# owensgroup/sparsify.me

Hardware: AMD Instinct MI355X
Metric: effective GF/s (2:4 spmma vs dense gemm) on ResNet-50 layer shapes (higher is better)
Workload: dtype f16

## Files before the change

sparsify.me_amd/csrc/spmma_f16_fused.hip:

```cpp
#include "select24.h"
#include "spmma_args.h"

namespace sm {

constexpr int MAXG = 8;
struct FusedArgs {
  const half_t* A[MAXG];
  const half_t* B[MAXG];
  half_t* C[MAXG];
  size_t sA, sB, sC;
  int Mrows, N, K, lda;
  int batch, tiles_m, tiles_n;
  int ngroup;
  float alpha, beta;
  const half_t* const* dAp;
  const half_t* const* dBp;
  half_t* const* dCp;
};

struct FusedArgsEpi : FusedArgs {
  EpiArgs e;
};
template <bool EPI> struct FusedArgsSel { typedef FusedArgs type; };
template <> struct FusedArgsSel<true> { typedef FusedArgsEpi type; };
// ... 568 lines not shown
  const int m0 = (int)tile_m * BM, n0 = (int)tile_n * BN;
  const int nkt = (p.K + 63) / 64;
  const char* A = reinterpret_cast<const char*>(p.dAp ? p.dAp[grp] : p.A[grp]);
  const half_t* B = p.dBp ? p.dBp[grp] : p.B[grp];
  half_t* C = p.dCp ? p.dCp[grp] : p.C[grp];
  const unsigned rowbytes = (unsigned)p.K * 2u;
  const int rows = p.Mrows - m0 < BM ? p.Mrows - m0 : BM;
  EpiBias<FM, FN> eb;
  if constexpr (EPI) eb = epi_bias_prefetch<FM, FN>(p.e, true, wave * TM, 0, m0, n0, p.Mrows, p.N, lane);

  {
    const size_t s0 = (size_t)m0 * rowbytes;
    const unsigned len = (unsigned)rows * rowbytes;
    const unsigned np = (len + 1023u) / 1024u;
    const size_t last16 = a_bytes - 16;
    for (unsigned pc = wave; pc < np; pc += NW) {
      size_t off = s0 + (size_t)pc * 1024u + 16u * lane;
      off = off < last16 ? off : last16;
      __builtin_amdgcn_global_load_lds((gptr_t*)(A + off), (lptr_t*)(smem + pc * 1024u), 16, 0, 2);
    }
  }
  char* const Bimg = smem + span_lds;
  {
    constexpr int B_N = BN / 8;
    const int npb = nkt * B_N;
    for (int t = (int)wave; t < npb; t += NW) {
      const int kt = t / B_N, j = t - kt * B_N;
      const unsigned panel = (unsigned)j >> 3, kr = 8u * ((unsigned)j & 7u) + (lane >> 3);
      const unsigned cs = (lane & 7u) ^ b_swz(kr);
      int gc = n0 + (int)(64u * panel + 8u * cs);
      gc = gc <= p.N - 8 ? gc : p.N - 8;
      const int krow = kt * 64 + (int)kr;
      const char* src = krow < p.K ? reinterpret_cast<const char*>(B + (size_t)krow * p.N + gc)
                                   : reinterpret_cast<const char*>(sm_fused_zero_page) + 16u * (lane & 7u);
      __builtin_amdgcn_global_load_lds((gptr_t*)src, (lptr_t*)(Bimg + kt * SB + panel * 8192u + ((unsigned)j & 7u) * 1024u), 16, 0, 0);
    }
  }
  wait_dma_and_barrier<0>();

  f4 acc[FM][FN];
#pragma unroll
  for (int i = 0; i < FM; ++i)
#pragma unroll
    for (int j = 0; j < FN; ++j) acc[i][j] = f4{0.f, 0.f, 0.f, 0.f};
  const unsigned g = lane >> 4, r = lane & 15u;
  unsigned rowoff[FM];
#pragma unroll
  for (int i = 0; i < FM; ++i) {
    int row = (int)(wave * TM + i * 16 + r);
    row = row < rows ? row : rows - 1;
    rowoff[i] = (unsigned)row * rowbytes;
  }
  for (int kt = 0; kt < nkt; ++kt) {
    if constexpr (DENSE) {
      h8 a0[FM], a1[FM];
#pragma unroll
      for (int i = 0; i < FM; ++i) {
        uint32_t d[2][4];
#pragma unroll
        for (int h = 0; h < 2; ++h) {
          const int k0 = kt * 64 + 32 * h + 8 * (int)g;
          int nv = p.K - k0;
          nv = nv < 0 ? 0 : (nv > 8 ? 8 : nv);
          const char* src = smem + rowoff[i] + 2u * (unsigned)k0;
#pragma unroll
          for (int e = 0; e < 4; ++e) {
            const uint32_t lo16 = *reinterpret_cast<const unsigned short*>(src + 4 * e);
            const uint32_t hi16 = *reinterpret_cast<const unsigned short*>(src + 4 * e + 2);
            uint32_t v = lo16 | (hi16 << 16);
            v = 2 * e + 1 < nv ? v : (2 * e < nv ? (v & 0xffffu) : 0u);
            d[h][e] = v;
          }
        }
        a0[i] = __builtin_bit_cast(h8, u4{d[0][0], d[0][1], d[0][2], d[0][3]});
        a1[i] = __builtin_bit_cast(h8, u4{d[1][0], d[1][1], d[1][2], d[1][3]});
      }
      mfma_b_sweep<FM, FN, BF>(a0, a1, Bimg + kt * SB, 0, lane, acc);
      continue;
    }
    h8 af[FM];
    int idx[FM];
    const int k0 = kt * 64 + 16 * (int)g;
    int nv = p.K - k0;
    nv = nv < 0 ? 0 : (nv > 16 ? 16 : nv);
#pragma unroll
    for (int i = 0; i < FM; ++i) {
      const char* src = smem + rowoff[i] + 2u * (unsigned)k0;
      uint32_t d[8];
#pragma unroll
      for (int e = 0; e < 8; ++e) {
        const uint32_t lo16 = *reinterpret_cast<const unsigned short*>(src + 4 * e);
        const uint32_t hi16 = *reinterpret_cast<const unsigned short*>(src + 4 * e + 2);
        uint32_t v = lo16 | (hi16 << 16);
        v = 2 * e + 1 < nv ? v : (2 * e < nv ? (v & 0xffffu) : 0u);
        d[e] = v;
      }
      dense16_to_operand(u4{d[0], d[1], d[2], d[3]}, u4{d[4], d[5], d[6], d[7]}, af[i], idx[i]);
    }
    smfmac_b_sweep<FM, FN, BF>(af, idx, Bimg + kt * SB, 0, lane, acc);
  }
  __syncthreads();
  if constexpr (EPI) store_c_tile_epi<BM, BN, FM, FN, 64 * NW, BF>(smem, C, p.e.R, p.e, eb, acc, true, wave * TM, 0, m0, n0, p.Mrows, p.N, p.alpha, p.beta, tid);
  else store_c_tile<BM, BN, FM, FN, 64 * NW, BF>(smem, C, acc, true, wave * TM, 0, m0, n0, p.Mrows, p.N, p.alpha, p.beta, tid);
}

template <int BN, bool BF = false, bool DENSE = false, bool EPI = false>
static int launch_fused_span(const typename FusedArgsSel<EPI>::type& a0, hipStream_t st) {
  typename FusedArgsSel<EPI>::type a = a0;
  a.tiles_m = (a.Mrows + 127) / 128;
  a.tiles_n = (a.N + BN - 1) / BN;
  const size_t nwg = (size_t)a.tiles_m * a.tiles_n * a.ngroup;
  if (nwg == 0) return SM_STATUS_SUCCESS;
  const size_t kc = ((size_t)a.K + 63) / 64 * 64;
  const size_t span_lds = ((size_t)128 * a.K * 2 + 128 + 1023) / 1024 * 1024;
  const size_t lds_main = span_lds + kc * BN * 2;
  constexpr size_t lds_epi = (size_t)128 * (BN * 2 + 16);
  const size_t lds = lds_main > lds_epi ? lds_main : lds_epi;
  if (lds > 160 * 1024 || nwg > 0x7fffffffu) {
    set_error("sm_spmma_fused_{f16,bf16}: k too long for the span form (use the staged path)");
    return SM_STATUS_NOT_SUPPORTED;
  }
  static LdsOptIn lds_optin;
  if (const int rc = ensure_dyn_lds(lds_optin, reinterpret_cast<const void*>(&spmma_f16_fused_span_kernel<BN, BF, DENSE, EPI>), 160 * 1024, "spmma_f16_fused_span_kernel")) return rc;
  spmma_f16_fused_span_kernel<BN, BF, DENSE, EPI><<<dim3((unsigned)nwg), dim3(256), lds, st>>>(a, (unsigned)span_lds, (size_t)a.Mrows * a.K * 2);
  return check_launch("spmma_f16_fused_span_kernel");
}

template <int BN, int NBW>
struct BTileDma {
  static constexpr int B_WI = (BN / 8) / NBW;
  const char* src[B_WI];
  unsigned dst[B_WI];
  size_t step;
  __device__ __forceinline__ void setup(const half_t* B, int N, int n0, unsigned bw, unsigned lane, unsigned ring_off) {
#pragma unroll
    for (int i = 0; i < B_WI; ++i) {
      const unsigned j = bw + (unsigned)NBW * i, panel = j >> 3, grp = j & 7u, kr = 8u * grp + (lane >> 3);
      const unsigned cs = (lane & 7u) ^ b_swz(kr);
      int gc = n0 + (int)(64u * panel + 8u * cs);
      gc = gc <= N - 8 ? gc : N - 8;
      src[i] = reinterpret_cast<const char*>(B) + ((size_t)kr * N + (size_t)gc) * 2;
      dst[i] = ring_off + panel * 8192u + grp * 1024u;
    }
    step = (size_t)64 * N * 2;
  }
  __device__ __forceinline__ void issue(char* smem, int kt, unsigned buf_off) const {
#pragma unroll
    for (int i = 0; i < B_WI; ++i)
      __builtin_amdgcn_global_load_lds((gptr_t*)(src[i] + (size_t)kt * step), (lptr_t*)(smem + buf_off + dst[i]), 16, 0, 0);
  }
};


template <int BN, int WM, int WN, int NLB, int PF, int NSB, bool BF = false, bool ANT = true, bool EPI = false>
__global__ __launch_bounds__(64 * (WM * WN + 4 + NLB)) void spmma_f16_fused_wide_kernel(const typename FusedArgsSel<EPI>::type p) {
  constexpr int BM = 128, NLA = 4, NC = WM * WN, NW = NC + NLA + NLB;
  static_assert(PF >= 1 && PF <= 3 && NSB >= 2 && NSB <= 4, "pipeline depths");
  constexpr int TM = BM / WM, TN = BN / WN, FM = TM / 16, FN = TN / 16;
  constexpr int SA = BM * 64, SM_ = BM * 8, ASTG = SA + SM_, SB = 64 * BN * 2;
  constexpr int BRING = 2 * ASTG;
  constexpr int NBW = NLB > 0 ? NLB : WM * WN;
  constexpr int B_N = BN / 8, B_WI = B_N / NBW;
  static_assert(B_N % NBW == 0 && B_WI >= 1 && (NSB - 2) * B_WI <= 63, "B tile vs issuing waves");
  extern __shared__ __attribute__((aligned(16))) char smem[];

  const unsigned tid = threadIdx.x, lane = tid & 63u;
  const unsigned wave = __builtin_amdgcn_readfirstlane(tid >> 6);
  const unsigned tiles = (unsigned)p.tiles_m * (unsigned)p.tiles_n;
  const unsigned lid = xcd_remap(blockIdx.x, gridDim.x);
  const unsigned gb = lid / tiles, trem = lid - gb * tiles;
  const unsigned grp = gb / (unsigned)p.batch, b = gb - grp * (unsigned)p.batch;
  const unsigned tile_m = trem / (unsigned)p.tiles_n, tile_n = trem - tile_m * (unsigned)p.tiles_n;
  const int m0 = (int)tile_m * BM, n0 = (int)tile_n * BN;
  const int nkt = p.K / 64;
  half_t* C = p.C[grp] + (size_t)b * p.sC;

  f4 acc[FM][FN];
#pragma unroll
  for (int i = 0; i < FM; ++i)
#pragma unroll
    for (int j = 0; j < FN; ++j) acc[i][j] = f4{0.f, 0.f, 0.f, 0.f};
  const unsigned wm = wave / WN, wn = wave % WN;
  EpiBias<FM, FN> eb;
  if constexpr (EPI) eb = epi_bias_prefetch<FM, FN>(p.e, wave < (unsigned)NC, wm * TM, wn * TN, m0, n0, p.Mrows, p.N, lane);

  if (NLB > 0 && wave >= (unsigned)(NC + NLA)) {
    BTileDma<BN, NBW> bd;
    bd.setup(p.B[grp] + (size_t)b * p.sB, p.N, n0, wave - (NC + NLA), lane, BRING);
    auto issue = [&](int kt, int buf) {
      bd.issue(smem, kt, (unsigned)(buf * SB));
    };
#pragma unroll
    for (int s = 0; s < NSB - 1; ++s)
      if (s < nkt) issue(s, s);
    int nb = NSB - 1;
    for (int kt = 0; kt < nkt; ++kt) {
      if (kt + NSB - 2 < nkt) wait_dma_and_barrier<(NSB - 2) * B_WI>();
      else wait_dma_and_barrier<0>();
      if (kt + NSB - 1 < nkt) {
        issue(kt + NSB - 1, nb);
        nb = nb + 1 == NSB ? 0 : nb + 1;
      }
    }
  } else if (wave >= (unsigned)NC) {
    const unsigned lw = wave - NC;
    const half_t* A = p.A[grp] + (size_t)b * p.sA;
    const int mlast = p.Mrows - 1;
    const unsigned c8 = lane & 7u;
    const half_t* a_src[4];
    unsigned a_val_off[4], a_meta_off[4];
#pragma unroll
    for (int i = 0; i < 4; ++i) {
      const unsigned row = 8u * (4u * lw + i) + (lane >> 3);
      int gr = m0 + (int)row;
      gr = gr < mlast ? gr : mlast;
      a_src[i] = A + (size_t)gr * p.lda + 8u * c8;
      a_val_off[i] = row * 64u + 16u * ((c8 >> 1) ^ a64_swz(row)) + 8u * (c8 & 1u);
      a_meta_off[i] = SA + row * 8u + c8;
    }
    u4 ra[PF][4];
    auto load_a = [&](int kt, u4 (&dst)[4]) {
#pragma unroll
      for (int i = 0; i < 4; ++i) {
        if constexpr (ANT) dst[i] = __builtin_nontemporal_load(reinterpret_cast<const u4*>(a_src[i] + (size_t)kt * 64));
        else dst[i] = *reinterpret_cast<const u4*>(a_src[i] + (size_t)kt * 64);
      }
      __builtin_amdgcn_sched_barrier(0);
    };
    auto write_stage = [&](int kt, const u4 (&src)[4]) {
      char* sb = smem + (kt & 1) * ASTG;
#pragma unroll
      for (int i = 0; i < 4; ++i) {
        uint32_t k0, k1, n0, n1;
        strip_select_f16(src[i][0], src[i][1], k0, n0);
        strip_select_f16(src[i][2], src[i][3], k1, n1);
        *reinterpret_cast<u2*>(sb + a_val_off[i]) = u2{k0, k1};
        *reinterpret_cast<unsigned char*>(sb + a_meta_off[i]) = (unsigned char)(n0 | (n1 << 4));
      }
    };
    auto step = [&](int kt, u4 (&rr)[4], bool write, bool load) {
      asm volatile("s_waitcnt lgkmcnt(0)\n\ts_barrier" ::: "memory");
      __builtin_amdgcn_sched_barrier(0);
      if (write) {
        write_stage(kt + 1, rr);
      }
      if (load) load_a(kt + 1 + PF, rr);
      __builtin_amdgcn_sched_barrier(0);
    };
    int kt0 = 0;
    if (nkt > 2 * PF) {
#pragma unroll
      for (int s = 0; s < PF; ++s) load_a(s, ra[s]);
      write_stage(0, ra[0]);
      load_a(PF, ra[0]);
      for (; kt0 + 2 * PF < nkt; kt0 += PF) {
#pragma unroll
        for (int u = 0; u < PF; ++u) step(kt0 + u, ra[(u + 1) % PF], true, true);
      }
    } else {
#pragma unroll
      for (int s = 0; s < PF; ++s)
        if (s < nkt) load_a(s, ra[s]);
      write_stage(0, ra[0]);
      if (PF < nkt) load_a(PF, ra[0]);
    }
    for (; kt0 < nkt; kt0 += PF) {
#pragma unroll
      for (int u = 0; u < PF; ++u) {
        const int kt = kt0 + u;
        if (kt < nkt) step(kt, ra[(u + 1) % PF], kt + 1 < nkt, kt + 1 + PF < nkt);
      }
    }
  } else {
    int cb = 0;
    BTileDma<BN, NBW> bd;
    int nb = NSB - 1;
    if (NLB == 0) {
      bd.setup(p.B[grp] + (size_t)b * p.sB, p.N, n0, wave, lane, BRING);
#pragma unroll
      for (int s = 0; s < NSB - 1; ++s)
        if (s < nkt) bd.issue(smem, s, (unsigned)(s * SB));
    }
    for (int kt = 0; kt < nkt; ++kt) {
      if (NLB == 0) {
        if (kt + NSB - 2 < nkt) wait_dma_and_barrier<(NSB - 2) * B_WI>();
        else wait_dma_and_barrier<0>();
        if (kt + NSB - 1 < nkt) {
          bd.issue(smem, kt + NSB - 1, (unsigned)(nb * SB));
          nb = nb + 1 == NSB ? 0 : nb + 1;
        }
      } else {
        wait_dma_and_barrier<0>();
      }
      const char* As = smem + (kt & 1) * ASTG;
      const char* Ms = As + SA;
      const char* Bs = smem + BRING + cb * SB;
      smfmac_stage<FM, FN, BF>(As, Ms, Bs, wm * TM, wn * TN, lane, acc);
      cb = cb + 1 == NSB ? 0 : cb + 1;
    }
  }
  __syncthreads();

  if constexpr (EPI) store_c_tile_epi<BM, BN, FM, FN, 64 * NW, BF>(smem, C, p.e.R + (size_t)b * p.e.sR, p.e, eb, acc, wave < (unsigned)NC, wm * TM, wn * TN, m0, n0, p.Mrows, p.N, p.alpha, p.beta, tid);
  else store_c_tile<BM, BN, FM, FN, 64 * NW, BF>(smem, C, acc, wave < (unsigned)NC, wm * TM, wn * TN, m0, n0, p.Mrows, p.N, p.alpha, p.beta, tid);
}

template <int BN, int WM, int WN, int NLB, int PF, int NSB, bool BF = false, bool ANT = true, bool EPI = false>
static int launch_fused_wide(const typename FusedArgsSel<EPI>::type& a0, hipStream_t st) {
  typename FusedArgsSel<EPI>::type a = a0;
  a.tiles_m = (a.Mrows + 127) / 128;
  a.tiles_n = (a.N + BN - 1) / BN;
  const size_t nwg = (size_t)a.tiles_m * a.tiles_n * a.batch * a.ngroup;
  if (nwg == 0) return SM_STATUS_SUCCESS;
  if (nwg > 0x7fffffffu) {
    set_error("sm_spmma_fused_f16: grid too large");
    return SM_STATUS_NOT_SUPPORTED;
  }
  constexpr size_t lds_main = 2 * (size_t)128 * 72 + (size_t)NSB * 64 * BN * 2;
  constexpr size_t lds_epi = (size_t)128 * (BN * 2 + 16);
  constexpr size_t lds = lds_main > lds_epi ? lds_main : lds_epi;
  static LdsOptIn lds_optin;
  if (lds > 64 * 1024) {
    if (const int rc = ensure_dyn_lds(lds_optin, reinterpret_cast<const void*>(&spmma_f16_fused_wide_kernel<BN, WM, WN, NLB, PF, NSB, BF, ANT, EPI>), lds, "spmma_f16_fused_wide_kernel")) return rc;
  }
  spmma_f16_fused_wide_kernel<BN, WM, WN, NLB, PF, NSB, BF, ANT, EPI><<<dim3((unsigned)nwg), dim3(64 * (WM * WN + 4 + NLB)), lds, st>>>(a);
  return check_launch("spmma_f16_fused_wide_kernel");
}

template <int BN, int WM, int WN, int NLB, int PF, int NSB, bool BF = false>
__global__ __launch_bounds__(64 * (WM * WN + 4 + NLB)) void spmma_f16_fused_widep_kernel(const FusedArgs p, const unsigned total) {
  constexpr int BM = 128, NLA = 4, NC = WM * WN;
  static_assert(NLB > 0 && PF >= 1 && PF <= 3 && NSB >= 2 && NSB <= 4, "pipeline depths");
  constexpr int TM = BM / WM, TN = BN / WN, FM = TM / 16, FN = TN / 16;
  static_assert(TN == 128 && TM == 32, "epilogue patch geometry");
  constexpr int SA = BM * 64, SM_ = BM * 8, ASTG = SA + SM_, SB = 64 * BN * 2;
  constexpr int BRING = 2 * ASTG;
  constexpr int B_N = BN / 8, B_WI = B_N / NLB;
  static_assert(B_N % NLB == 0 && (NSB - 2) * B_WI <= 63, "B tile vs loader waves");
  constexpr int WPITCH = 64 * 2 + 8, WPATCH = TM * WPITCH;
  constexpr int CPATCH = BRING + NSB * SB;
  extern __shared__ __attribute__((aligned(16))) char smem[];

  const unsigned tid = threadIdx.x, lane = tid & 63u;
  const unsigned wave = __builtin_amdgcn_readfirstlane(tid >> 6);
  const unsigned tiles = (unsigned)p.tiles_m * (unsigned)p.tiles_n;
  const int nkt = p.K / 64;
  const unsigned my_tiles = (total - blockIdx.x + gridDim.x - 1u) / gridDim.x;
  const int S = (int)my_tiles * nkt;

  struct Tile {
    unsigned grp, b;
    int m0, n0;
  };
  auto tile_of = [&](unsigned j) {
    Tile t;
    const unsigned lid = xcd_remap(blockIdx.x + j * gridDim.x, total);
    const unsigned gb = lid / tiles, trem = lid - gb * tiles;
    t.grp = gb / (unsigned)p.batch;
    t.b = gb - t.grp * (unsigned)p.batch;
    const unsigned tile_m = trem / (unsigned)p.tiles_n, tile_n = trem - tile_m * (unsigned)p.tiles_n;
    t.m0 = (int)tile_m * BM;
    t.n0 = (int)tile_n * BN;
    return t;
  };

  if (wave >= (unsigned)(NC + NLA)) {
    BTileDma<BN, NLB> bd;
    unsigned ij = 0;
    int ikt = 0, nb = 0;
    {
      const Tile t = tile_of(0);
      bd.setup(p.B[t.grp] + (size_t)t.b * p.sB, p.N, t.n0, wave - (NC + NLA), lane, BRING);
    }
    auto issue = [&]() {
      bd.issue(smem, ikt, (unsigned)(nb * SB));
      nb = nb + 1 == NSB ? 0 : nb + 1;
      if (++ikt == nkt) {
        ikt = 0;
        if (++ij < my_tiles) {
          const Tile t = tile_of(ij);
          bd.setup(p.B[t.grp] + (size_t)t.b * p.sB, p.N, t.n0, wave - (NC + NLA), lane, BRING);
        }
      }
    };
#pragma unroll
    for (int s = 0; s < NSB - 1; ++s)
      if (s < S) issue();
    for (int g = 0; g < S; ++g) {
      if (g + NSB - 2 < S) wait_dma_and_barrier<(NSB - 2) * B_WI>();
      else wait_dma_and_barrier<0>();
      if (g + NSB - 1 < S) issue();
    }
  } else if (wave >= (unsigned)NC) {
    const unsigned lw = wave - NC;
    const unsigned c8 = lane & 7u;
    const half_t* a_src[4];
    unsigned a_val_off[4], a_meta_off[4];
#pragma unroll
    for (int i = 0; i < 4; ++i) {
      const unsigned row = 8u * (4u * lw + i) + (lane >> 3);
      a_val_off[i] = row * 64u + 16u * ((c8 >> 1) ^ a64_swz(row)) + 8u * (c8 & 1u);
      a_meta_off[i] = SA + row * 8u + c8;
    }
    const int mlast = p.Mrows - 1;
    auto point_at = [&](unsigned j) {
      const Tile t = tile_of(j);
      const half_t* A = p.A[t.grp] + (size_t)t.b * p.sA;
#pragma unroll
      for (int i = 0; i < 4; ++i) {
        const unsigned row = 8u * (4u * lw + i) + (lane >> 3);
        int gr = t.m0 + (int)row;
        gr = gr < mlast ? gr : mlast;
        a_src[i] = A + (size_t)gr * p.lda + 8u * c8;
      }
    };
    point_at(0);
    unsigned lj = 0;
    int lkt = 0;
    u4 ra[PF][4];
    auto load_a = [&](u4 (&dst)[4]) {
#pragma unroll
      for (int i = 0; i < 4; ++i) dst[i] = __builtin_nontemporal_load(reinterpret_cast<const u4*>(a_src[i] + (size_t)lkt * 64));
      __builtin_amdgcn_sched_barrier(0);
      if (++lkt == nkt) {
        lkt = 0;
        if (++lj < my_tiles) point_at(lj);
      }
    };
    auto write_stage = [&](int g, const u4 (&src)[4]) {
      char* sb = smem + (g & 1) * ASTG;
#pragma unroll
      for (int i = 0; i < 4; ++i) {
        uint32_t k0, k1, n0, n1;
        strip_select_f16(src[i][0], src[i][1], k0, n0);
        strip_select_f16(src[i][2], src[i][3], k1, n1);
        *reinterpret_cast<u2*>(sb + a_val_off[i]) = u2{k0, k1};
        *reinterpret_cast<unsigned char*>(sb + a_meta_off[i]) = (unsigned char)(n0 | (n1 << 4));
      }
    };
    auto step = [&](int g, u4 (&rr)[4], bool write, bool load) {
      asm volatile("s_waitcnt lgkmcnt(0)\n\ts_barrier" ::: "memory");
      __builtin_amdgcn_sched_barrier(0);
      if (write) write_stage(g + 1, rr);
      if (load) load_a(rr);
      __builtin_amdgcn_sched_barrier(0);
    };
    int g0 = 0;
    if (S > 2 * PF) {
#pragma unroll
      for (int s = 0; s < PF; ++s) load_a(ra[s]);
      write_stage(0, ra[0]);
      load_a(ra[0]);
      for (; g0 + 2 * PF < S; g0 += PF) {
#pragma unroll
        for (int u = 0; u < PF; ++u) step(g0 + u, ra[(u + 1) % PF], true, true);
      }
    } else {
#pragma unroll
      for (int s = 0; s < PF; ++s)
        if (s < S) load_a(ra[s]);
      write_stage(0, ra[0]);
      if (PF < S) load_a(ra[0]);
    }
    for (; g0 < S; g0 += PF) {
#pragma unroll
      for (int u = 0; u < PF; ++u) {
        const int g = g0 + u;
        if (g < S) step(g, ra[(u + 1) % PF], g + 1 < S, g + 1 + PF < S);
      }
    }
  } else {
    const unsigned g4 = lane >> 4, r = lane & 15u;
    const unsigned wm = wave / WN, wn = wave % WN;
    char* const patch = smem + CPATCH + wave * WPATCH;
    f4 acc[FM][FN];
#pragma unroll
    for (int i = 0; i < FM; ++i)
#pragma unroll
// ... 263 lines not shown
using namespace sm;

static bool span_form_takes(size_t m, size_t n, size_t k, size_t lda, size_t batch, size_t strideA, size_t strideB, size_t strideC, bool all_aligned, bool c_aligned) {
  return (k % 64 != 0 || lda % 8 != 0) && lda == k && n % 8 == 0 && n <= 128 && all_aligned && c_aligned && (batch == 1 || (strideB == 0 && strideA == m * lda && strideC == m * n)) &&
         (m * batch * k * 2) % 16 == 0 && m * batch <= 0x7fffffffull && k <= 0x7fffffffull &&
         ((size_t)128 * k * 2 + 1152) + ((k + 63) / 64 * 64) * (n <= 64 ? 64 : 128) * 2 <= 160 * 1024;
}
static bool stage_forms_take(size_t n, size_t k, size_t lda, size_t strideA, size_t strideB, bool all_aligned) {
  return !(k % 64 != 0 || lda % 8 != 0 || strideA % 8 != 0 || n % 8 != 0 || strideB % 8 != 0 || !all_aligned);
}
static bool dims_fit_int(size_t m, size_t n, size_t k, size_t lda, size_t batch) {
  return !(m * batch > 0x7fffffffull || n > 0x7fffffffull || k > 0x7fffffffull || lda > 0x7fffffffull);
}

struct FusedCall {
  size_t m, n, k, lda, batch, count, sA, sB, sC;
  float beta;
  bool a_aligned, b_aligned, c_aligned;
  bool ws, ws_aligned;
  size_t ws_bytes;
  bool epi, r_aligned;
  size_t sR;
};
struct FusedPick {
  int form;
  bool stacked;
  const char* why;
};

static FusedPick fused_form(const FusedCall& c, size_t cus) {
  const size_t m = c.m, n = c.n, k = c.k, lda = c.lda, batch = c.batch;
  if (c.count == 0 || m == 0 || n == 0 || batch == 0) return {SM_FUSED_FORM_EMPTY, false, nullptr};
  const bool all_aligned = c.a_aligned && c.b_aligned;
  const bool contiguous = c.sB == 0 && c.sA == m * lda && c.sC == m * n;
  if (n < 8 && k <= 64 && lda == k && (batch == 1 || contiguous)) {
    if (c.epi) return {SM_FUSED_FORM_NOT_TAKEN, false, "sm_spmma_fused_{f16,bf16}_ex: the thin form (n < 8) takes no epilogue"};
    if (thin_form_takes(c.count, m * batch, n, k) && c.a_aligned) return {SM_FUSED_FORM_THIN, true, nullptr};
  }
  const bool r_follows = !c.epi || c.beta == 0.0f || (c.r_aligned && (batch == 1 || c.sR == m * n));
  if (span_form_takes(m, n, k, lda, batch, c.sA, c.sB, c.sC, all_aligned, c.c_aligned && r_follows)) return {SM_FUSED_FORM_SPAN, true, nullptr};
  if (!stage_forms_take(n, k, lda, c.sA, c.sB, all_aligned))
    return {SM_FUSED_FORM_NOT_TAKEN, false, "sm_spmma_fused_{f16,bf16}: needs k % 64 == 0, n % 8 == 0 and 16-byte aligned rows (use the staged path)"};
  if (c.count > 1 && !c.c_aligned)
    return {SM_FUSED_FORM_NOT_TAKEN, false, "sm_spmma_fused_{f16,bf16}_grouped: needs 16-byte aligned C operands"};
  if (!dims_fit_int(m, n, k, lda, batch)) return {SM_FUSED_FORM_NOT_TAKEN, false, "sm_spmma_fused_{f16,bf16}: dimension exceeds 2^31-1"};
  const bool stacked = batch > 1 && contiguous && (!c.epi || c.beta == 0.0f || c.sR == m * n);
  const size_t rows = stacked ? m * batch : m, nb = (stacked ? 1 : batch) * c.count;
  const bool astat_store = n > 256 && k <= 512 && c.beta == 0.0f && c.c_aligned && (c.sC % 8 == 0);
  if (c.ws) {
    SkPlan pl;
    if (sk_takes(rows, nb, n, k, astat_store, cus, pl) && c.ws_bytes >= sk_workspace_bytes((size_t)pl.slots * ((n + 255) / 256), 256) && c.ws_aligned &&
        !sk_launch_limits((rows + 255) / 256 * nb, n, k, lda, cus))
      return {SM_FUSED_FORM_STREAMK, stacked, nullptr};
  }
  auto round_eff = [](size_t tiles, size_t cus_) { const size_t r = (tiles + cus_ - 1) / cus_; return r ? (double)tiles / (double)(r * cus_) : 1.0; };
  if (n > 128 && k > 64) {
    const size_t t_big = (rows + 255) / 256 * ((n + 255) / 256) * nb, t_wide = (rows + 127) / 128 * ((n + 255) / 256) * nb;
    bool big = round_eff(t_big, cus) >= round_eff(t_wide, cus);
    if (!c.epi && astat_store) {
      const size_t panels = (rows + 127) / 128 * nb;
      big = round_eff(t_big, cus) > round_eff(panels * astat_nsplit(panels, (n + 127) / 128, cus), cus) + 0.1;
    }
    if (big) return {SM_FUSED_FORM_BIG, stacked, nullptr};
  }
  if (n <= 128 || (n <= 256 && k <= 64)) {
    if (n <= 64) return {SM_FUSED_FORM_DIRECT64, stacked, nullptr};
    return {n > 128 || k < 512 ? SM_FUSED_FORM_DIRECT128 : SM_FUSED_FORM_DIRECT128_NT, stacked, nullptr};
  }
  if (!c.epi && astat_store && astat_lds_bytes((int)(k / 64), 3) <= 160 * 1024) return {SM_FUSED_FORM_ASTAT, stacked, nullptr};
  if (k <= 1024 && !c.epi) return {SM_FUSED_FORM_WIDEP, stacked, nullptr};
  return {n > 256 ? SM_FUSED_FORM_WIDE : SM_FUSED_FORM_WIDE_NT, stacked, nullptr};
}

static bool fused_form_is_exact(int form) { return form != SM_FUSED_FORM_NOT_TAKEN && form != SM_FUSED_FORM_EMPTY && form != SM_FUSED_FORM_THIN; }

bool sm::spmma_fused16_takes_exact(const void* A, const void* B, const void* C, size_t m, size_t n, size_t k, size_t lda, size_t batch, size_t strideA, size_t strideB,
                                   size_t strideC) {
  if (!A || !B || !C || lda < k) return false;
  const FusedCall c = {m, n, k, lda, batch, 1, strideA, strideB, strideC, 0.0f, aligned16(A), aligned16(B), aligned16(C), false, false, 0, false, false, 0};
  return fused_form_is_exact(fused_form(c, 256).form);
}

extern "C" int sm_spmma_fused_form(size_t m, size_t n, size_t k, size_t lda, size_t batch, size_t count, size_t strideA, size_t strideB, size_t strideC,
                                   float beta, unsigned flags, size_t cus, int* form) {
  constexpr unsigned known = SM_FUSED_FLAG_A_ALIGNED | SM_FUSED_FLAG_B_ALIGNED | SM_FUSED_FLAG_C_ALIGNED | SM_FUSED_FLAG_WORKSPACE | SM_FUSED_FLAG_EPILOGUE;
  if (!form || lda < k || count > (size_t)MAXG || (flags & ~known) || ((flags & SM_FUSED_FLAG_WORKSPACE) && (flags & SM_FUSED_FLAG_EPILOGUE))) {
    set_error("sm_spmma_fused_form: invalid argument");
    return SM_STATUS_INVALID_VALUE;
  }
  const bool c_al = (flags & SM_FUSED_FLAG_C_ALIGNED) != 0, ws = (flags & SM_FUSED_FLAG_WORKSPACE) != 0;
  const FusedCall c = {m, n, k, lda, batch, count, strideA, strideB, strideC, beta, (flags & SM_FUSED_FLAG_A_ALIGNED) != 0, (flags & SM_FUSED_FLAG_B_ALIGNED) != 0, c_al,
                       ws, ws, ws ? ~(size_t)0 : 0, (flags & SM_FUSED_FLAG_EPILOGUE) != 0, c_al, strideC};
  *form = fused_form(c, cus ? cus : (size_t)device_cu_count()).form;
  return SM_STATUS_SUCCESS;
}

template <bool BF>
static int spmma_fused16(size_t ngroup, const void* const* Ag, const void* const* Bg, void* const* Cg, size_t m, size_t n, size_t k, size_t lda,
                         size_t batch, size_t strideA, size_t strideB, size_t strideC, float alpha, float beta,
                         sm_stream_t stream, void* workspace = nullptr, size_t workspace_bytes = 0, const EpiArgs* epi = nullptr) {
#define SM_LAUNCH(fn, ...) (epi ? fn<__VA_ARGS__, true>(ae, st) : fn<__VA_ARGS__, false>(a, st))
  if (ngroup == 0) return SM_STATUS_SUCCESS;
  if (!Ag || !Bg || !Cg || lda < k || ngroup > (size_t)MAXG) {
    set_error("sm_spmma_fused_{f16,bf16}: invalid argument");
    return SM_STATUS_INVALID_VALUE;
  }
  FusedCall c = {m, n, k, lda, batch, ngroup, strideA, strideB, strideC, beta, true, true, true, workspace != nullptr, aligned16(workspace), workspace_bytes,
                 epi != nullptr, epi && aligned16(epi->R), epi ? epi->sR : 0};
  for (size_t g = 0; g < ngroup; ++g) {
    if (!Ag[g] || !Bg[g] || !Cg[g]) {
      set_error("sm_spmma_fused_{f16,bf16}: invalid argument (null operand)");
      return SM_STATUS_INVALID_VALUE;
    }
    c.a_aligned = c.a_aligned && aligned16(Ag[g]);
    c.b_aligned = c.b_aligned && aligned16(Bg[g]);
    c.c_aligned = c.c_aligned && aligned16(Cg[g]);
  }
  const FusedPick pick = fused_form(c, (size_t)device_cu_count());
  hipStream_t st = (hipStream_t)stream;
  FusedArgs a = {};
  for (size_t g = 0; g < (size_t)MAXG; ++g) {
    const size_t s_ = g < ngroup ? g : 0;
    a.A[g] = (const half_t*)Ag[s_]; a.B[g] = (const half_t*)Bg[s_]; a.C[g] = (half_t*)Cg[s_];
  }
  a.ngroup = (int)ngroup;
  a.N = (int)n; a.K = (int)k; a.lda = (int)lda;
  a.alpha = alpha; a.beta = beta;
  if (pick.stacked) {
    a.Mrows = (int)(m * batch);
    a.batch = 1;
  } else {
    a.Mrows = (int)m;
    a.batch = (int)batch;
  }
  if (pick.form != SM_FUSED_FORM_SPAN) { a.sA = strideA; a.sB = strideB; a.sC = strideC; }
  FusedArgsEpi ae = {};
  static_cast<FusedArgs&>(ae) = a;
  if (epi) ae.e = *epi;
  switch (pick.form) {
    case SM_FUSED_FORM_EMPTY: return SM_STATUS_SUCCESS;
    case SM_FUSED_FORM_NOT_TAKEN:
      set_error("%s", pick.why);
      return SM_STATUS_NOT_SUPPORTED;
    case SM_FUSED_FORM_THIN: return spmma_fused_thin(BF, (int)ngroup, Ag, Bg, Cg, m * batch, n, k, alpha, beta, st);
    case SM_FUSED_FORM_SPAN: return n <= 64 ? SM_LAUNCH(launch_fused_span, 64, BF, false) : SM_LAUNCH(launch_fused_span, 128, BF, false);
    case SM_FUSED_FORM_STREAMK:
      return n <= 256 ? launch_fused_sk<256, BF, true>(a, workspace, workspace_bytes, st) : launch_fused_sk<256, BF, false>(a, workspace, workspace_bytes, st);
    case SM_FUSED_FORM_BIG: return n <= 256 ? SM_LAUNCH(launch_fused_big, 256, BF, 3, 2, true, false) : SM_LAUNCH(launch_fused_big, 256, BF, 3, 2, false, false);
    case SM_FUSED_FORM_DIRECT64: return SM_LAUNCH(launch_fused_direct, 64, 2, BF, 128, 4, true, false);
    case SM_FUSED_FORM_DIRECT128: return SM_LAUNCH(launch_fused_direct, 128, 2, BF, 128, 4, false, false);
    case SM_FUSED_FORM_DIRECT128_NT: return SM_LAUNCH(launch_fused_direct, 128, 2, BF, 128, 4, true, false);
    case SM_FUSED_FORM_ASTAT: return launch_fused_astat<BF>(a, st);
    case SM_FUSED_FORM_WIDEP: return launch_fused_widep<256, 4, 2, 4, 2, 3, BF>(a, st);
    case SM_FUSED_FORM_WIDE: return SM_LAUNCH(launch_fused_wide, 256, 4, 2, 4, 2, 3, BF, false);
    case SM_FUSED_FORM_WIDE_NT: return SM_LAUNCH(launch_fused_wide, 256, 4, 2, 4, 2, 3, BF, true);
  }
  set_error("sm_spmma_fused_{f16,bf16}: internal error (unknown form)");
  return SM_STATUS_LAUNCH_FAILED;
#undef SM_LAUNCH
}

extern "C" int sm_spmma_fused_f16(const void* A, const void* B, void* C, size_t m, size_t n, size_t k, size_t lda,
                                  size_t batch, size_t strideA, size_t strideB, size_t strideC, float alpha, float beta,
                                  sm_stream_t stream) {
  return spmma_fused16<false>(1, &A, &B, &C, m, n, k, lda, batch, strideA, strideB, strideC, alpha, beta, stream);
}
extern "C" int sm_spmma_fused_bf16(const void* A, const void* B, void* C, size_t m, size_t n, size_t k, size_t lda,
                                   size_t batch, size_t strideA, size_t strideB, size_t strideC, float alpha, float beta,
                                   sm_stream_t stream) {
  return spmma_fused16<true>(1, &A, &B, &C, m, n, k, lda, batch, strideA, strideB, strideC, alpha, beta, stream);
}

template <bool BF>
static int spmma_fused16_ex(const void* A, const void* B, void* D, size_t m, size_t n, size_t k, size_t lda, size_t batch, size_t strideA, size_t strideB,
                            size_t strideD, float alpha, float beta, const sm_epilogue_t* ep, sm_stream_t stream) {
  EpiArgs e;
  bool plain;
  if (const int rc = epilogue_args(ep, D, strideD, m, beta, e, &plain, "sm_spmma_fused_{f16,bf16}_ex")) return rc;
  return spmma_fused16<BF>(1, &A, &B, &D, m, n, k, lda, batch, strideA, strideB, strideD, alpha, beta, stream, nullptr, 0, plain ? nullptr : &e);
}
extern "C" int sm_spmma_fused_f16_ex(const void* A, const void* B, void* D, size_t m, size_t n, size_t k, size_t lda, size_t batch,
                                     size_t strideA, size_t strideB, size_t strideD, float alpha, float beta, const sm_epilogue_t* epilogue,
                                     sm_stream_t stream) {
  return spmma_fused16_ex<false>(A, B, D, m, n, k, lda, batch, strideA, strideB, strideD, alpha, beta, epilogue, stream);
}
extern "C" int sm_spmma_fused_bf16_ex(const void* A, const void* B, void* D, size_t m, size_t n, size_t k, size_t lda, size_t batch,
                                      size_t strideA, size_t strideB, size_t strideD, float alpha, float beta, const sm_epilogue_t* epilogue,
                                      sm_stream_t stream) {
  return spmma_fused16_ex<true>(A, B, D, m, n, k, lda, batch, strideA, strideB, strideD, alpha, beta, epilogue, stream);
}

extern "C" int sm_spmma_fused_workspace_size(size_t* bytes) {
  if (!bytes) {
    set_error("sm_spmma_fused_workspace_size: invalid argument");
    return SM_STATUS_INVALID_VALUE;
  }
  *bytes = sk_workspace_bytes((size_t)device_cu_count(), 256);
  return SM_STATUS_SUCCESS;
}
extern "C" int sm_spmma_fused_workspace_state(const void* workspace, int* state, sm_stream_t stream) {
  if (!workspace || !state) {
    set_error("sm_spmma_fused_workspace_state: invalid argument");
    return SM_STATUS_INVALID_VALUE;
  }
  unsigned h[1024];
  hipStream_t st = (hipStream_t)stream;
  if (hipMemcpyAsync(h, workspace, sizeof(h), hipMemcpyDeviceToHost, st) != hipSuccess || hipStreamSynchronize(st) != hipSuccess)
    return check_launch("sm_spmma_fused_workspace_state");
  bool dirty = false;
  for (int i = 0; i < 1023; ++i) dirty = dirty || h[i] != 0u;
  *state = h[1023] != 0u ? 1 : (dirty ? 2 : 0);
  return SM_STATUS_SUCCESS;
}
extern "C" int sm_spmma_fused_streamk_plan(size_t rows, size_t n, size_t k, size_t problems, int* takes, unsigned* plan) {
  if (!takes || !plan) {
    set_error("sm_spmma_fused_streamk_plan: invalid argument");
    return SM_STATUS_INVALID_VALUE;
  }
  SkPlan pl = {};
  *takes = sk_takes(rows, problems, n, k, n > 256 && k <= 512, (size_t)device_cu_count(), pl) ? 1 : 0;
  unsigned* o = plan;
  *o++ = pl.tg; *o++ = pl.wg; *o++ = pl.groups_full; *o++ = pl.tgl; *o++ = pl.wgl; *o++ = pl.slots; *o++ = pl.units;
  for (int i = 0; i < 9; ++i) *o++ = pl.cut[i];
  for (int i = 0; i < 9; ++i) *o++ = pl.cutl[i];
  return SM_STATUS_SUCCESS;
}
extern "C" int sm_spmma_fused_f16_ws(const void* A, const void* B, void* C, size_t m, size_t n, size_t k, size_t lda, size_t batch, size_t strideA,
                                     size_t strideB, size_t strideC, float alpha, float beta, void* workspace, size_t workspace_bytes, sm_stream_t stream) {
  return spmma_fused16<false>(1, &A, &B, &C, m, n, k, lda, batch, strideA, strideB, strideC, alpha, beta, stream, workspace, workspace_bytes);
}
extern "C" int sm_spmma_fused_bf16_ws(const void* A, const void* B, void* C, size_t m, size_t n, size_t k, size_t lda, size_t batch, size_t strideA,
                                      size_t strideB, size_t strideC, float alpha, float beta, void* workspace, size_t workspace_bytes, sm_stream_t stream) {
  return spmma_fused16<true>(1, &A, &B, &C, m, n, k, lda, batch, strideA, strideB, strideC, alpha, beta, stream, workspace, workspace_bytes);
}

template <bool BF>
static int dense_twin16(const DenseTwinCall& c, hipStream_t st) {
  const size_t n = (size_t)c.N, k = (size_t)c.K;
  const bool tables = c.Ap != nullptr;
  if (tables != (c.Bp != nullptr) || tables != (c.Cp != nullptr)) return SM_STATUS_NOT_SUPPORTED;
  if (c.N % 8 != 0 || c.N < 8 || (!tables && (!aligned16(c.A) || !aligned16(c.B) || !aligned16(c.C)))) return SM_STATUS_NOT_SUPPORTED;
  FusedArgs a = {};
  for (int g = 0; g < MAXG; ++g) { a.A[g] = c.A; a.B[g] = c.B; a.C[g] = c.C; }
  a.dAp = c.Ap; a.dBp = c.Bp; a.dCp = c.Cp;
  a.ngroup = 1;
  a.sA = c.sA; a.sB = c.sB; a.sC = c.sC;
  a.Mrows = c.M; a.N = c.N; a.K = c.K; a.lda = c.lda;
  a.batch = c.batch; a.alpha = c.alpha; a.beta = c.beta;
  if (k % 64 != 0 || c.lda % 8 != 0) {
    if (c.lda != c.K || n > 128 || ((size_t)c.M * k * 2) % 16 != 0 || (c.batch > 1 && !tables)) return SM_STATUS_NOT_SUPPORTED;
    if (((size_t)128 * k * 2 + 1152) + ((k + 63) / 64 * 64) * (n <= 64 ? 64 : 128) * 2 > 160 * 1024) return SM_STATUS_NOT_SUPPORTED;
    a.ngroup = c.batch;
    a.batch = 1;
    if (!tables) a.ngroup = 1;
    return n <= 64 ? launch_fused_span<64, BF, true>(a, st) : launch_fused_span<128, BF, true>(a, st);
  }
  if (c.sA % 8 != 0 || c.sB % 8 != 0) return SM_STATUS_NOT_SUPPORTED;
  if (c.workspace && n > 128 && n <= 256 && k >= 2048) {
    SkPlan pl;
    if (sk_takes((size_t)c.M, (size_t)c.batch, n, k, false, (size_t)device_cu_count(), pl) && c.workspace_bytes >= sk_workspace_bytes((size_t)pl.slots * ((n + 255) / 256), 256) &&
        aligned16(c.workspace))
      return launch_fused_sk<256, BF, true, true>(a, c.workspace, c.workspace_bytes, st);
  }
  if (n <= 128) return SM_STATUS_NOT_SUPPORTED;
  if (k <= 64) return SM_STATUS_NOT_SUPPORTED;
  if (((size_t)c.M + 255) / 256 * 256 * 100 > (size_t)c.M * 115) return SM_STATUS_NOT_SUPPORTED;
  if (!(n <= 256 && k >= 2048)) return SM_STATUS_NOT_SUPPORTED;
  return launch_fused_big<256, BF, 3, 2, true, true>(a, st);
}

int sm::gemm_dense_twin(const DenseTwinCall& c, hipStream_t st) { return c.bf ? dense_twin16<true>(c, st) : dense_twin16<false>(c, st); }

template <bool BF>
static int spmma_fused16_grouped(size_t count, const void* const* A, const void* const* B, void* const* C, size_t m, size_t n, size_t k,
                                 size_t lda, size_t batch, size_t strideA, size_t strideB, size_t strideC, float alpha, float beta,
                                 sm_stream_t stream, void* workspace = nullptr, size_t workspace_bytes = 0) {
  if (count && (!A || !B || !C)) {
    set_error("sm_spmma_fused_{f16,bf16}_grouped: invalid argument");
    return SM_STATUS_INVALID_VALUE;
  }
  for (size_t i = 0; i < count; i += (size_t)MAXG) {
    const size_t ng = count - i < (size_t)MAXG ? count - i : (size_t)MAXG;
    if (const int rc = spmma_fused16<BF>(ng, A + i, B + i, C + i, m, n, k, lda, batch, strideA, strideB, strideC, alpha, beta, stream, workspace, workspace_bytes)) return rc;
  }
  return SM_STATUS_SUCCESS;
}
extern "C" int sm_spmma_fused_f16_grouped(size_t count, const void* const* A, const void* const* B, void* const* C, size_t m, size_t n,
                                          size_t k, size_t lda, size_t batch, size_t strideA, size_t strideB, size_t strideC,
                                          float alpha, float beta, sm_stream_t stream) {
  return spmma_fused16_grouped<false>(count, A, B, C, m, n, k, lda, batch, strideA, strideB, strideC, alpha, beta, stream);
}
extern "C" int sm_spmma_fused_bf16_grouped(size_t count, const void* const* A, const void* const* B, void* const* C, size_t m, size_t n,
                                           size_t k, size_t lda, size_t batch, size_t strideA, size_t strideB, size_t strideC,
                                           float alpha, float beta, sm_stream_t stream) {
  return spmma_fused16_grouped<true>(count, A, B, C, m, n, k, lda, batch, strideA, strideB, strideC, alpha, beta, stream);
}
extern "C" int sm_spmma_fused_f16_grouped_ws(size_t count, const void* const* A, const void* const* B, void* const* C, size_t m, size_t n,
                                             size_t k, size_t lda, size_t batch, size_t strideA, size_t strideB, size_t strideC,
                                             float alpha, float beta, void* workspace, size_t workspace_bytes, sm_stream_t stream) {
  return spmma_fused16_grouped<false>(count, A, B, C, m, n, k, lda, batch, strideA, strideB, strideC, alpha, beta, stream, workspace, workspace_bytes);
}
extern "C" int sm_spmma_fused_bf16_grouped_ws(size_t count, const void* const* A, const void* const* B, void* const* C, size_t m, size_t n,
                                              size_t k, size_t lda, size_t batch, size_t strideA, size_t strideB, size_t strideC,
                                              float alpha, float beta, void* workspace, size_t workspace_bytes, sm_stream_t stream) {
  return spmma_fused16_grouped<true>(count, A, B, C, m, n, k, lda, batch, strideA, strideB, strideC, alpha, beta, stream, workspace, workspace_bytes);
}
```

Measured before the change: 576,700.

## Parameterize A-loader wave count; move B DMA issue after MMA in wide kernel

```diff
diff --git a/sparsify.me_amd/csrc/spmma_f16_fused.hip b/sparsify.me_amd/csrc/spmma_f16_fused.hip
--- a/sparsify.me_amd/csrc/spmma_f16_fused.hip
+++ b/sparsify.me_amd/csrc/spmma_f16_fused.hip
@@ -744,9 +744,11 @@
 };
 
 
-template <int BN, int WM, int WN, int NLB, int PF, int NSB, bool BF = false, bool ANT = true, bool EPI = false>
-__global__ __launch_bounds__(64 * (WM * WN + 4 + NLB)) void spmma_f16_fused_wide_kernel(const typename FusedArgsSel<EPI>::type p) {
-  constexpr int BM = 128, NLA = 4, NC = WM * WN, NW = NC + NLA + NLB;
+template <int BN, int WM, int WN, int NLA, int NLB, int PF, int NSB, bool BF = false, bool ANT = true, bool EPI = false>
+__global__ __launch_bounds__(64 * (WM * WN + NLA + NLB)) void spmma_f16_fused_wide_kernel(const typename FusedArgsSel<EPI>::type p) {
+  constexpr int BM = 128, NC = WM * WN, NW = NC + NLA + NLB;
+  constexpr int A_WI = 16 / NLA;
+  static_assert((NLA == 4 || NLA == 8) && NW <= 16, "A loader waves");
   static_assert(PF >= 1 && PF <= 3 && NSB >= 2 && NSB <= 4, "pipeline depths");
   constexpr int TM = BM / WM, TN = BN / WN, FM = TM / 16, FN = TN / 16;
   constexpr int SA = BM * 64, SM_ = BM * 8, ASTG = SA + SM_, SB = 64 * BN * 2;
@@ -799,30 +801,30 @@
     const half_t* A = p.A[grp] + (size_t)b * p.sA;
     const int mlast = p.Mrows - 1;
     const unsigned c8 = lane & 7u;
-    const half_t* a_src[4];
-    unsigned a_val_off[4], a_meta_off[4];
-#pragma unroll
-    for (int i = 0; i < 4; ++i) {
-      const unsigned row = 8u * (4u * lw + i) + (lane >> 3);
+    const half_t* a_src[A_WI];
+    unsigned a_val_off[A_WI], a_meta_off[A_WI];
+#pragma unroll
+    for (int i = 0; i < A_WI; ++i) {
+      const unsigned row = 8u * ((unsigned)A_WI * lw + i) + (lane >> 3);
       int gr = m0 + (int)row;
       gr = gr < mlast ? gr : mlast;
       a_src[i] = A + (size_t)gr * p.lda + 8u * c8;
       a_val_off[i] = row * 64u + 16u * ((c8 >> 1) ^ a64_swz(row)) + 8u * (c8 & 1u);
       a_meta_off[i] = SA + row * 8u + c8;
     }
-    u4 ra[PF][4];
-    auto load_a = [&](int kt, u4 (&dst)[4]) {
-#pragma unroll
-      for (int i = 0; i < 4; ++i) {
+    u4 ra[PF][A_WI];
+    auto load_a = [&](int kt, u4 (&dst)[A_WI]) {
+#pragma unroll
+      for (int i = 0; i < A_WI; ++i) {
         if constexpr (ANT) dst[i] = __builtin_nontemporal_load(reinterpret_cast<const u4*>(a_src[i] + (size_t)kt * 64));
         else dst[i] = *reinterpret_cast<const u4*>(a_src[i] + (size_t)kt * 64);
       }
       __builtin_amdgcn_sched_barrier(0);
     };
-    auto write_stage = [&](int kt, const u4 (&src)[4]) {
+    auto write_stage = [&](int kt, const u4 (&src)[A_WI]) {
       char* sb = smem + (kt & 1) * ASTG;
 #pragma unroll
-      for (int i = 0; i < 4; ++i) {
+      for (int i = 0; i < A_WI; ++i) {
         uint32_t k0, k1, n0, n1;
         strip_select_f16(src[i][0], src[i][1], k0, n0);
         strip_select_f16(src[i][2], src[i][3], k1, n1);
@@ -830,7 +832,7 @@
         *reinterpret_cast<unsigned char*>(sb + a_meta_off[i]) = (unsigned char)(n0 | (n1 << 4));
       }
     };
-    auto step = [&](int kt, u4 (&rr)[4], bool write, bool load) {
+    auto step = [&](int kt, u4 (&rr)[A_WI], bool write, bool load) {
       asm volatile("s_waitcnt lgkmcnt(0)\n\ts_barrier" ::: "memory");
       __builtin_amdgcn_sched_barrier(0);
       if (write) {
@@ -874,20 +876,16 @@
         if (s < nkt) bd.issue(smem, s, (unsigned)(s * SB));
     }
     for (int kt = 0; kt < nkt; ++kt) {
-      if (NLB == 0) {
-        if (kt + NSB - 2 < nkt) wait_dma_and_barrier<(NSB - 2) * B_WI>();
-        else wait_dma_and_barrier<0>();
-        if (kt + NSB - 1 < nkt) {
-          bd.issue(smem, kt + NSB - 1, (unsigned)(nb * SB));
-          nb = nb + 1 == NSB ? 0 : nb + 1;
-        }
-      } else {
-        wait_dma_and_barrier<0>();
-      }
+      if (NLB == 0 && kt + NSB - 2 < nkt) wait_dma_and_barrier<(NSB - 2) * B_WI>();
+      else wait_dma_and_barrier<0>();
       const char* As = smem + (kt & 1) * ASTG;
       const char* Ms = As + SA;
       const char* Bs = smem + BRING + cb * SB;
       smfmac_stage<FM, FN, BF>(As, Ms, Bs, wm * TM, wn * TN, lane, acc);
+      if (NLB == 0 && kt + NSB - 1 < nkt) {
+        bd.issue(smem, kt + NSB - 1, (unsigned)(nb * SB));
+        nb = nb + 1 == NSB ? 0 : nb + 1;
+      }
       cb = cb + 1 == NSB ? 0 : cb + 1;
     }
   }
@@ -897,7 +895,7 @@
   else store_c_tile<BM, BN, FM, FN, 64 * NW, BF>(smem, C, acc, wave < (unsigned)NC, wm * TM, wn * TN, m0, n0, p.Mrows, p.N, p.alpha, p.beta, tid);
 }
 
-template <int BN, int WM, int WN, int NLB, int PF, int NSB, bool BF = false, bool ANT = true, bool EPI = false>
+template <int BN, int WM, int WN, int NLA, int NLB, int PF, int NSB, bool BF = false, bool ANT = true, bool EPI = false>
 static int launch_fused_wide(const typename FusedArgsSel<EPI>::type& a0, hipStream_t st) {
   typename FusedArgsSel<EPI>::type a = a0;
   a.tiles_m = (a.Mrows + 127) / 128;
@@ -913,9 +911,9 @@
   constexpr size_t lds = lds_main > lds_epi ? lds_main : lds_epi;
   static LdsOptIn lds_optin;
   if (lds > 64 * 1024) {
-    if (const int rc = ensure_dyn_lds(lds_optin, reinterpret_cast<const void*>(&spmma_f16_fused_wide_kernel<BN, WM, WN, NLB, PF, NSB, BF, ANT, EPI>), lds, "spmma_f16_fused_wide_kernel")) return rc;
-  }
-  spmma_f16_fused_wide_kernel<BN, WM, WN, NLB, PF, NSB, BF, ANT, EPI><<<dim3((unsigned)nwg), dim3(64 * (WM * WN + 4 + NLB)), lds, st>>>(a);
+    if (const int rc = ensure_dyn_lds(lds_optin, reinterpret_cast<const void*>(&spmma_f16_fused_wide_kernel<BN, WM, WN, NLA, NLB, PF, NSB, BF, ANT, EPI>), lds, "spmma_f16_fused_wide_kernel")) return rc;
+  }
+  spmma_f16_fused_wide_kernel<BN, WM, WN, NLA, NLB, PF, NSB, BF, ANT, EPI><<<dim3((unsigned)nwg), dim3(64 * (WM * WN + NLA + NLB)), lds, st>>>(a);
   return check_launch("spmma_f16_fused_wide_kernel");
 }
 
@@ -1485,8 +1483,8 @@
     case SM_FUSED_FORM_DIRECT128_NT: return SM_LAUNCH(launch_fused_direct, 128, 2, BF, 128, 4, true, false);
     case SM_FUSED_FORM_ASTAT: return launch_fused_astat<BF>(a, st);
     case SM_FUSED_FORM_WIDEP: return launch_fused_widep<256, 4, 2, 4, 2, 3, BF>(a, st);
-    case SM_FUSED_FORM_WIDE: return SM_LAUNCH(launch_fused_wide, 256, 4, 2, 4, 2, 3, BF, false);
-    case SM_FUSED_FORM_WIDE_NT: return SM_LAUNCH(launch_fused_wide, 256, 4, 2, 4, 2, 3, BF, true);
+    case SM_FUSED_FORM_WIDE: return epi ? launch_fused_wide<256, 4, 2, 4, 4, 2, 3, BF, false, true>(ae, st) : launch_fused_wide<256, 4, 2, 8, 0, 3, 3, BF, false, false>(a, st);
+    case SM_FUSED_FORM_WIDE_NT: return SM_LAUNCH(launch_fused_wide, 256, 4, 2, 4, 4, 2, 3, BF, true);
   }
   set_error("sm_spmma_fused_{f16,bf16}: internal error (unknown form)");
   return SM_STATUS_LAUNCH_FAILED;
```

After: 575,100. No clear change (-0.3%).
